# Alexandre-nk-Perdereau/video-fingerprint

Measured on NVIDIA B200. Metric: fingerprint videos/s (64 frames@64^2), higher is better.
Workload: dtype bf16

## Files before the change

### video_fingerprint_b200/csrc/ffn_kernel.cuh

```cuda
#pragma once
#include "epilogues.cuh"
#include "sm100_primitives.cuh"

namespace vfp {

constexpr int kFfnHidden = 1024;
constexpr int kFfnChunk = 256;
constexpr int kFfnChunks = kFfnHidden / kFfnChunk;
constexpr int kFfnActWarps = 16;
constexpr int kFfnThreads = 64 + 32 * kFfnActWarps;

#ifdef VFP_FFN_TRACE
__device__ long long g_ffn_trace[8192];
__device__ unsigned int g_ffn_trace_n = 0;
#define FFN_TRACE_DECL(role) int trace_i = 0; const int trace_role = (role); (void)trace_i; (void)trace_role
#define FFN_TRACE(tag) do { if (blockIdx.x == 0 && trace_i < 1024) { g_ffn_trace[(trace_role * 1024 + trace_i) * 2] = (tag); g_ffn_trace[(trace_role * 1024 + trace_i) * 2 + 1] = clock64(); ++trace_i; } } while (0)
#else
#define FFN_TRACE_DECL(role)
#define FFN_TRACE(tag)
#endif

template <int SLOTS>
struct FfnSmem {
  static constexpr int kA0 = 0;
  static constexpr int kRing = kA0 + 4 * 16384;
  static constexpr int kH = kRing + SLOTS * 16384;
  static constexpr int kBias = kH + 4 * 16384;
  static constexpr int kBars = kBias + 5 * 1024;
  static constexpr int kTotal = kBars + 512 + 1024;
};

struct FfnParams {
  alignas(64) CUtensorMap tmap_x;
  alignas(64) CUtensorMap tmap_w1;
  alignas(64) CUtensorMap tmap_w2;
  alignas(64) CUtensorMap tmap_out;
  const float* b1;
  const float* b2;
  int M;
  int pair_tiles;
};

template <int SLOTS>
__global__ void __launch_bounds__(kFfnThreads, 1) ffn_pair_kernel(const __grid_constant__ FfnParams p) {
  using L = FfnSmem<SLOTS>;
  static_assert(L::kTotal <= 232448, "ffn kernel shared memory");
  extern __shared__ uint8_t smem_raw[];
  uint8_t* smem = smem_raw + ((1024u - (smem_u32(smem_raw) & 1023u)) & 1023u);
  uint8_t* a0 = smem + L::kA0;
  uint8_t* ring = smem + L::kRing;
  uint8_t* hbuf = smem + L::kH;
  float* sbias = reinterpret_cast<float*>(smem + L::kBias);
  uint64_t* bars = reinterpret_cast<uint64_t*>(smem + L::kBars);
  uint64_t* full = bars;
  uint64_t* empty = bars + SLOTS;
  uint64_t* a0_full = bars + 2 * SLOTS;
  uint64_t* a0_empty = a0_full + 1;
  uint64_t* d1_full = a0_full + 2;
  uint64_t* d1_empty = a0_full + 3;
  uint64_t* h_full = a0_full + 4;
  uint64_t* h_empty = a0_full + 5;
  uint64_t* d2_full = a0_full + 6;
  uint64_t* d2_empty = a0_full + 7;
  uint32_t* tmem_slot = reinterpret_cast<uint32_t*>(a0_full + 8);

  const int warp = threadIdx.x >> 5, lane = threadIdx.x & 31;
  const uint32_t crank = cluster_ctarank();
  const bool leader = crank == 0;
  const int pair = blockIdx.x >> 1, n_pairs = gridDim.x >> 1;
  const int my_tiles = p.pair_tiles > pair ? (p.pair_tiles - pair + n_pairs - 1) / n_pairs : 0;
  const int n_chunks = my_tiles * kFfnChunks;
  pdl_launch_dependents();

  if (warp == 0 && lane == 0) {
    tma_prefetch_desc(&p.tmap_x);
    tma_prefetch_desc(&p.tmap_w1);
    tma_prefetch_desc(&p.tmap_w2);
    tma_prefetch_desc(&p.tmap_out);
    for (int i = 0; i < SLOTS; ++i) {
      mbar_init(&full[i], 1);
      mbar_init(&empty[i], 1);
    }
    mbar_init(a0_full, 1);
    mbar_init(a0_empty, 1);
    mbar_init(d1_full, 1);
    mbar_init(d1_empty, 2 * kFfnActWarps);
    mbar_init(h_full, 2 * kFfnActWarps);
    mbar_init(h_empty, 1);
    mbar_init(d2_full, 1);
    mbar_init(d2_empty, 2 * kFfnActWarps);
    fence_mbar_init();
  }
  if (warp == 1) {
    tmem_alloc_2cta(tmem_slot, 512);
    tmem_relinquish_2cta();
  }
  uint32_t* sbias_h = reinterpret_cast<uint32_t*>(sbias);
  for (int i = threadIdx.x; i < kFfnHidden / 2; i += kFfnThreads) {
    const __half2 h = __floats2half2_rn(__ldg(p.b1 + 2 * i), __ldg(p.b1 + 2 * i + 1));
    sbias_h[i] = *reinterpret_cast<const uint32_t*>(&h);
  }
  for (int i = threadIdx.x; i < 256; i += kFfnThreads) sbias[kFfnHidden + i] = __ldg(p.b2 + i);
  tc_fence_before();
  __syncthreads();
  cluster_sync_all();
  tc_fence_after();
  const uint32_t tmem_base = *tmem_slot;
  pdl_wait();

  if (warp == 0) {
    if (lane == 0) {
      int slot = 0;
      uint32_t ph = 0, a_ph = 0;
      const uint32_t a0_full_leader = mapa_u32(a0_full, 0);
      auto load_w = [&](const CUtensorMap* map, int k_col, int row0) {
        mbar_wait(&empty[slot], ph ^ 1);
        if (leader) mbar_arrive_expect_tx(&full[slot], 2 * 16384);
        tma_load_2d_2cta(map, mapa_u32(&full[slot], 0), ring + slot * 16384, k_col, row0 + (int)crank * 128);
        if (++slot == SLOTS) { slot = 0; ph ^= 1; }
      };
      auto load_g1 = [&](int n) {
        const int c = n % kFfnChunks;
        if (c == 0) {
          const int tile = pair + (n / kFfnChunks) * n_pairs;
          mbar_wait(a0_empty, a_ph ^ 1);
          a_ph ^= 1;
          if (leader) mbar_arrive_expect_tx(a0_full, 2 * 4 * 16384);
          for (int kb = 0; kb < 4; ++kb) tma_load_2d_2cta(&p.tmap_x, a0_full_leader, a0 + kb * 16384, kb * 64, (tile * 2 + (int)crank) * 128);
        }
        for (int kb = 0; kb < 4; ++kb) load_w(&p.tmap_w1, kb * 64, c * kFfnChunk);
      };
      auto load_g2 = [&](int n) {
        const int c = n % kFfnChunks;
        for (int kb = 0; kb < 4; ++kb) load_w(&p.tmap_w2, c * kFfnChunk + kb * 64, 0);
      };
      if (n_chunks > 0) load_g1(0);
      for (int n = 0; n < n_chunks; ++n) {
        if (n + 1 < n_chunks) load_g1(n + 1);
// ... 21 lines not shown
        mbar_wait(d1_empty, d1e_ph ^ 1);
        d1e_ph ^= 1;
        tc_fence_after();
        FFN_TRACE(101);
        for (int kb = 0; kb < 4; ++kb) {
          mbar_wait(&full[slot], ph);
          tc_fence_after();
          const uint64_t adesc = umma_smem_desc_kmajor<128>(a0_addr + kb * 16384);
          const uint64_t bdesc = umma_smem_desc_kmajor<128>(smem_u32(ring + slot * 16384));
#pragma unroll
          for (int k = 0; k < 4; ++k) umma_bf16_2cta(tmem_base, adesc + 2 * k, bdesc + 2 * k, idesc, (kb | k) != 0 ? 1u : 0u);
          commit_slot();
        }
        umma_commit_2cta(d1_full, 3);
        FFN_TRACE(102);
        if (c == kFfnChunks - 1) umma_commit_2cta(a0_empty, 3);
      };
      auto gemm2 = [&](int n) {
        const int c = n % kFfnChunks;
        if (c == 0) {
          mbar_wait(d2_empty, d2e_ph ^ 1);
          d2e_ph ^= 1;
        }
        FFN_TRACE(110);
        mbar_wait(h_full, hf_ph);
        hf_ph ^= 1;
        tc_fence_after();
        FFN_TRACE(111);
        for (int kb = 0; kb < 4; ++kb) {
          mbar_wait(&full[slot], ph);
          tc_fence_after();
// ... 52 lines not shown
      tc_fence_before();
      __syncwarp();
      if (lane == 0) mbar_arrive_cluster(d2_empty_leader);
      fence_proxy_async_smem();
      __syncwarp();
      if (lane == 0) {
        const int grow0 = (tile * 2 + (int)crank) * 128 + q * 32;
        tma_store_2d(&p.tmap_out, stage, cq * 64, grow0);
        tma_store_2d(&p.tmap_out, stage + 2048, cq * 64 + 32, grow0);
        tma_store_commit();
        tma_store_wait_read<0>();
      }
      asm volatile("bar.sync 1, %0;" ::"n"(32 * kFfnActWarps) : "memory");
    };

    for (int n = 0; n < n_chunks; ++n) {
      const int c = n % kFfnChunks;
      if (warp == 2 && lane == 0) FFN_TRACE(200);
      mbar_wait(d1_full, d1f_ph);
      d1f_ph ^= 1;
      tc_fence_after();
      if (warp == 2 && lane == 0) FFN_TRACE(201);
      uint32_t packed[32];
      {
        uint32_t va[32], vb[32];
        tmem_ld_32x32(lane_addr + cq * 64, va);
        tmem_ld_32x32(lane_addr + cq * 64 + 32, vb);
        tmem_ld_wait();
        if (warp == 2 && lane == 0) FFN_TRACE(203);
        tc_fence_before();
        __syncwarp();
        if (lane == 0) mbar_arrive_cluster(d1_empty_leader);
#pragma unroll
        for (int cc = 0; cc < 2; ++cc) {
          uint32_t(&v)[32] = cc ? vb : va;
          const uint32_t* bias = sbias_h + (c * kFfnChunk + cq * 64 + cc * 32) / 2;
// ... 41 lines not shown
```

### video_fingerprint_b200/csrc/sm100_primitives.cuh

```cuda
#pragma once
#include <cuda.h>
#include <cuda_runtime.h>
#include <cuda_bf16.h>
#include <stdint.h>

namespace vfp {

__device__ __forceinline__ uint32_t smem_u32(const void* p) {
  return static_cast<uint32_t>(__cvta_generic_to_shared(p));
}

__device__ __forceinline__ bool elect_one() {
  uint32_t pred = 0;
  asm volatile(
      "{\n\t"
      ".reg .pred P;\n\t"
      "elect.sync _|P, 0xffffffff;\n\t"
      "selp.u32 %0, 1, 0, P;\n\t"
      "}\n"
      : "=r"(pred));
  return pred != 0;
}

__device__ __forceinline__ void pdl_launch_dependents() { asm volatile("griddepcontrol.launch_dependents;" ::: "memory"); }
// ... 181 lines not shown
      "l"(adesc), "l"(bdesc), "r"(idesc), "r"(accumulate)
      : "memory");
}
__device__ __forceinline__ void umma_commit_2cta(uint64_t* bar, uint16_t cta_mask) {
  asm volatile("tcgen05.commit.cta_group::2.mbarrier::arrive::one.shared::cluster.multicast::cluster.b64 [%0], %1;" ::"r"(smem_u32(bar)),
               "h"(cta_mask)
               : "memory");
}

__device__ __forceinline__ void tma_prefetch_l2_2d(const CUtensorMap* m, int c0, int c1) {
  asm volatile("cp.async.bulk.prefetch.tensor.2d.L2.global.tile [%0, {%1, %2}];" ::"l"(reinterpret_cast<uint64_t>(m)), "r"(c0),
               "r"(c1)
               : "memory");
}

__device__ __forceinline__ void tma_store_2d(const CUtensorMap* m, const void* src, int c0, int c1) {
  asm volatile("cp.async.bulk.tensor.2d.global.shared::cta.bulk_group [%0, {%2, %3}], [%1];" ::"l"(
                   reinterpret_cast<uint64_t>(m)),
               "r"(smem_u32(src)), "r"(c0), "r"(c1)
               : "memory");
}
__device__ __forceinline__ void tma_store_commit() { asm volatile("cp.async.bulk.commit_group;" ::: "memory"); }
template <int N>
__device__ __forceinline__ void tma_store_wait_read() {
  asm volatile("cp.async.bulk.wait_group.read %0;" ::"n"(N) : "memory");
}

__device__ __forceinline__ void tmem_alloc(uint32_t* slot_in_smem, uint32_t ncols) {
  asm volatile("tcgen05.alloc.cta_group::1.sync.aligned.shared::cta.b32 [%0], %1;" ::"r"(smem_u32(slot_in_smem)),
               "r"(ncols)
// ... 116 lines not shown
```

### video_fingerprint_b200/csrc/stem_common.cuh

```cuda
#pragma once
#include "conv1_kernel.cuh"
#include "epilogues.cuh"

namespace vfp {

constexpr int kStemThreads = 768;
constexpr int kStemEpiWarp0 = 4, kStemEpiWarps = 8;
constexpr int kStemABuf = 9 * 16 * 128;
constexpr int kStemUnitBytes = 2 * kStemABuf;
constexpr int kStemWBlocks = 5;
constexpr int kStemRawSlotBytes = 8192;
constexpr int kStemTilePitch = 72;
constexpr int kStemTileBytes = 29184;
static_assert((67 * kStemTilePitch + 8) * 6 <= kStemTileBytes, "HWC tile");

template <int N> __device__ __forceinline__ void setmaxnreg_inc() { asm volatile("setmaxnreg.inc.sync.aligned.u32 %0;" ::"n"(N)); }
template <int N> __device__ __forceinline__ void setmaxnreg_dec() { asm volatile("setmaxnreg.dec.sync.aligned.u32 %0;" ::"n"(N)); }

__device__ __forceinline__ uint32_t relu_pack_bf16x2(float lo, float hi) {
  uint32_t d;
  asm("cvt.rn.relu.bf16x2.f32 %0, %1, %2;" : "=r"(d) : "f"(hi), "f"(lo));
  return d;
}
__device__ __forceinline__ void bulk_copy_g2s(void* dst, const void* src, uint32_t bytes, uint64_t* bar) {
  asm volatile("cp.async.bulk.shared::cluster.global.mbarrier::complete_tx::bytes [%0], [%1], %2, [%3];" ::"r"(smem_u32(dst)),
               "l"(reinterpret_cast<uint64_t>(src)), "r"(bytes), "r"(smem_u32(bar))
               : "memory");
}
__device__ __forceinline__ void bulk_prefetch_l2(const void* src, uint32_t bytes) {
  asm volatile("cp.async.bulk.prefetch.L2.global [%0], %1;" ::"l"(reinterpret_cast<uint64_t>(src)), "r"(bytes) : "memory");
}
__device__ __forceinline__ uint32_t u8x2_to_bf16x2(uint32_t lo, uint32_t hi) {
  return pack_bf16x2((float)lo * (1.0f / 255.0f), (float)hi * (1.0f / 255.0f));
}

__device__ __forceinline__ void stem_transpose_frame(const uint8_t* const (&pl)[3], uint8_t* tile, int frame_dtype, int ltid,
                                                     int n_threads) {
  if (frame_dtype == kFrameBF16) {
    for (int i = ltid; i < 512; i += n_threads) {
      const int h = i >> 3, w0 = (i & 7) * 8;
      const uint4 a = *reinterpret_cast<const uint4*>(pl[0] + (h * 64 + w0) * 2);
      const uint4 b = *reinterpret_cast<const uint4*>(pl[1] + (h * 64 + w0) * 2);
      const uint4 c = *reinterpret_cast<const uint4*>(pl[2] + (h * 64 + w0) * 2);
      uint4* dst = reinterpret_cast<uint4*>(tile + (h + 2) * (kStemTilePitch * 6) + (w0 + 8) * 6);
      uint4 o0, o1, o2;
// ... 53 lines not shown
```

### video_fingerprint_b200/csrc/token_kernels.cuh

```cuda
#pragma once
#include "sm100_primitives.cuh"
#include "epilogues.cuh"

namespace vfp {

constexpr int kDim = 256;
constexpr int kHeads = 8;
constexpr int kHeadDim = 32;

struct FrameSrc {
  unsigned long long addr;
  long long pitch;
};

__global__ void token_map_kernel(const int* __restrict__ cu, const FrameSrc* __restrict__ src, int n_clips, int n_tokens,
                                 int* __restrict__ tok_pos, int* __restrict__ tok_len, unsigned long long* __restrict__ frame_addr) {
  pdl_launch_dependents();
  pdl_wait();
  const int t = blockIdx.x * blockDim.x + threadIdx.x;
  if (t >= n_tokens) return;
  int lo = 0, hi = n_clips;
  while (hi - lo > 1) {
    const int mid = (lo + hi) >> 1;
    if (cu[mid] <= t) lo = mid; else hi = mid;
// ... 3 lines not shown
  tok_len[t] = cu[lo + 1] - cu[lo];
  const FrameSrc s = src[lo];
  frame_addr[t] = s.addr + (unsigned long long)((long long)pos * s.pitch);
}

__global__ void __launch_bounds__(256)
add_layernorm_bf16_kernel(float* __restrict__ x, const __nv_bfloat16* __restrict__ delta ,
                          const __nv_bfloat16* __restrict__ delta2 ,
                          const float* __restrict__ gamma, const float* __restrict__ beta, __nv_bfloat16* __restrict__ y,
                          int n_tokens, int write_x) {
  pdl_launch_dependents();
  pdl_wait();
  const int warp = (blockIdx.x * blockDim.x + threadIdx.x) >> 5;
  const int lane = threadIdx.x & 31;
  if (warp >= n_tokens) return;
  float4* xr = reinterpret_cast<float4*>(x + (size_t)warp * kDim) + lane * 2;
  const float4 a = xr[0], b = xr[1];
  float v[8] = {a.x, a.y, a.z, a.w, b.x, b.y, b.z, b.w};
  if (delta) {
    const uint4 d = reinterpret_cast<const uint4*>(delta + (size_t)warp * kDim)[lane];
    const __nv_bfloat162* dp = reinterpret_cast<const __nv_bfloat162*>(&d);
#pragma unroll
    for (int e = 0; e < 4; ++e) {
      const float2 f = __bfloat1622float2(dp[e]);
      v[2 * e] += f.x;
      v[2 * e + 1] += f.y;
    }
    if (delta2) {
      const uint4 d2 = reinterpret_cast<const uint4*>(delta2 + (size_t)warp * kDim)[lane];
      const __nv_bfloat162* dp2 = reinterpret_cast<const __nv_bfloat162*>(&d2);
#pragma unroll
      for (int e = 0; e < 4; ++e) {
        const float2 f = __bfloat1622float2(dp2[e]);
        v[2 * e] += f.x;
        v[2 * e + 1] += f.y;
      }
    }
    if (write_x) {
      xr[0] = make_float4(v[0], v[1], v[2], v[3]);
      xr[1] = make_float4(v[4], v[5], v[6], v[7]);
    }
  }
  float s = 0.f;
#pragma unroll
  for (int i = 0; i < 8; ++i) s += v[i];
#pragma unroll
  for (int o = 16; o > 0; o >>= 1) s += __shfl_xor_sync(0xffffffffu, s, o);
  const float mean = s * (1.0f / kDim);
  float q = 0.f;
#pragma unroll
  for (int i = 0; i < 8; ++i) { v[i] -= mean; q += v[i] * v[i]; }
#pragma unroll
  for (int o = 16; o > 0; o >>= 1) q += __shfl_xor_sync(0xffffffffu, q, o);
  const float rstd = rsqrtf(q * (1.0f / kDim) + 1e-5f);
  const float4 g0 = __ldg(reinterpret_cast<const float4*>(gamma) + lane * 2);
  const float4 g1 = __ldg(reinterpret_cast<const float4*>(gamma) + lane * 2 + 1);
  const float4 b0 = __ldg(reinterpret_cast<const float4*>(beta) + lane * 2);
  const float4 b1 = __ldg(reinterpret_cast<const float4*>(beta) + lane * 2 + 1);
  uint4 o;
  o.x = pack_bf16x2(v[0] * rstd * g0.x + b0.x, v[1] * rstd * g0.y + b0.y);
  o.y = pack_bf16x2(v[2] * rstd * g0.z + b0.z, v[3] * rstd * g0.w + b0.w);
  o.z = pack_bf16x2(v[4] * rstd * g1.x + b1.x, v[5] * rstd * g1.y + b1.y);
  o.w = pack_bf16x2(v[6] * rstd * g1.z + b1.z, v[7] * rstd * g1.w + b1.w);
  reinterpret_cast<uint4*>(y + (size_t)warp * kDim)[lane] = o;
}

__global__ void __launch_bounds__(256)
add_convert_bf16_kernel(float* __restrict__ x, const __nv_bfloat16* __restrict__ delta ,
                        const __nv_bfloat16* __restrict__ delta2 , __nv_bfloat16* __restrict__ xbf,
                        long long n8) {
  pdl_launch_dependents();
  pdl_wait();
  const long long i = (long long)blockIdx.x * blockDim.x + threadIdx.x;
  if (i >= n8) return;
  float4* xr = reinterpret_cast<float4*>(x) + 2 * i;
  const float4 a = xr[0], b = xr[1];
  float v[8] = {a.x, a.y, a.z, a.w, b.x, b.y, b.z, b.w};
  if (delta) {
    const uint4 d = reinterpret_cast<const uint4*>(delta)[i];
// ... 456 lines not shown
```

### video_fingerprint_b200/csrc/vfp_b200.cu

```cuda
#include "../../include/vfp_b200.h"

#include <math.h>
#include <string.h>

#include <map>
#include <mutex>
#include <string>
#include <vector>

#include "conv1_kernel.cuh"
#include "attention_tc_kernel.cuh"
#include "conv3_ts_kernel.cuh"
#include "ffn_kernel.cuh"
#include "gemm_launch.cuh"
#include "join_kernels.cuh"
#include "metrics_kernels.cuh"
#include "model3d_kernels.cuh"
#include "preprocess_kernels.cuh"
#include "stem_ts_kernel.cuh"
#include "token_kernels.cuh"
#include "topk_kernels.cuh"

using namespace vfp;

namespace {

thread_local std::string g_last_error;

int fail(const std::string& msg) {
  g_last_error = msg;
// ... 186 lines not shown
int prep_f32(vfp_weights* w, const float* src, size_t n, float** dev) {
  std::vector<float> v(src, src + n);
  return upload(w, v, dev);
}

constexpr int64_t kConvPassFrames = 262144;
constexpr int64_t kStemPassFrames = 16384;
int64_t g_conv_pass_frames = 65536;
int64_t g_stem_pass_frames = kStemPassFrames;
int g_fused_stem = 2;
int g_join_prefetch = 16;
int g_attention_tc = 1;
int g_conv3_ts = 1;
int g_pair_gemm = 1;
int g_ffn_mode = 1;
int g_conv_mcast = 0;
int g_join_kernel = 2;
int g_join_symmetric = 1;
int g_join_panel_tiles = 512;

struct TokenWs {
  size_t cu, frame_src, att_items, frame_addr, tok_pos, tok_len, feat, xa, xb, xn, qkv, att, delta, delta2, h, logits, xbf, pooled, pooled_bf, head_h, total;
};
struct ConvWs {
  size_t c1, c2, c3, total;
};
TokenWs token_ws_layout(int64_t F, int64_t C) {
  TokenWs L{};
  size_t off = 0;
  auto take = [&](size_t bytes) {
// ... 71 lines not shown
  int sms = 0;
  if (cudaDeviceGetAttribute(&sms, cudaDevAttrMultiProcessorCount, dev) != cudaSuccess) return 0;
  return sms;
}

int vfp_set_tuning(int key, long long value) {
  if (key == 0 && value >= 64 && value <= kStemPassFrames) { g_stem_pass_frames = value; return 0; }
  if (key == 1 && (value == 0 || value == 2)) { g_fused_stem = (int)value; return 0; }
  if (key == 5 && value >= 0 && value <= 4096) { g_join_prefetch = (int)value; return 0; }
  if (key == 6 && value >= 0 && value <= 4096) { g_topk_prefetch = (int)value; return 0; }
  if (key == 3 && value >= 64 && value <= kConvPassFrames) { g_conv_pass_frames = value; return 0; }
  if (key == 16 && value >= 0 && value <= 1) { g_conv3_ts = (int)value; return 0; }
  if (key == 17 && value >= 0 && value <= 1) { g_attention_tc = (int)value; return 0; }
  if (key == 15 && value >= 0 && value <= 3) { g_pair_gemm = (int)value; return 0; }
  if (key == 14 && value >= 0 && value <= 1) { g_ffn_mode = (int)value; return 0; }
  if (key == 13 && value >= 0 && value <= 3) { g_conv_mcast = (int)value; return 0; }
  if (key == 10 && value >= 0 && value <= 2) { g_join_kernel = (int)value; return 0; }
  if (key == 11 && value >= 0 && value <= 1) { g_join_symmetric = (int)value; return 0; }
  if (key == 12 && value >= 16 && value <= 65536) { g_join_panel_tiles = (int)value; return 0; }
  if (key == 7 && value >= 0 && value <= 1) { pdl_enabled().store((int)value); return 0; }
  if (key == 8 && value >= 0 && value <= 4096) { persistent_cta_limit().store((int)value); return 0; }
  if (key == 9 && value >= 1 && value <= kMaxPipes) { g_forward_pipes = (int)value; return 0; }
  if (key == 2) {
    const int mode = value != 0;
    const unsigned int zero = 0;
    if (cudaMemcpyToSymbol(g_vfp_hang_mode, &mode, sizeof(mode)) != cudaSuccess) return 2;
    if (cudaMemcpyToSymbol(g_vfp_hang_count, &zero, sizeof(zero)) != cudaSuccess) return 2;
    return 0;
  }
  return 1;
// ... 392 lines not shown

  std::vector<int32_t> cu_rel(C + 1);
  for (int i = 0; i <= C; ++i) cu_rel[i] = (int32_t)(cu_host[c0 + i] - f0);
  size_t n_items = 0;
  for (int i = 0; i < C; ++i) n_items += (size_t)(cu_rel[i + 1] - cu_rel[i] + kAttRows - 1) / kAttRows;
  std::vector<uint8_t> tables(L.att_items - L.cu + n_items * 16);
  memcpy(tables.data(), cu_rel.data(), (size_t)(C + 1) * 4);
  memcpy(tables.data() + (L.frame_src - L.cu), src + c0, (size_t)C * sizeof(FrameSrc));
  int32_t* items_host = reinterpret_cast<int32_t*>(tables.data() + (L.att_items - L.cu));
  for (int i = 0; i < C; ++i)
    for (int q = cu_rel[i]; q < cu_rel[i + 1]; q += kAttRows) {
      items_host[0] = q; items_host[1] = cu_rel[i]; items_host[2] = cu_rel[i + 1]; items_host[3] = 0;
      items_host += 4;
    }
  g_prof.mark(-1, st);
  g_prof.launches += 8 + 7 * (unsigned long long)w->n_attn;
  int4* att_items = reinterpret_cast<int4*>(ws + L.att_items);
  VFP_CUDA(cudaMemcpyAsync(d_cu, tables.data(), tables.size(), cudaMemcpyHostToDevice, st));
  VFP_CUDA(launch_kernel(token_map_kernel, dim3((unsigned)((F + 255) / 256)), dim3(256), 0, st, (const int*)d_cu, d_src, C, (int)F,
                         tok_pos, tok_len, frame_addr));
  g_prof.mark(kStMisc, st);

  for (int64_t s0 = 0; s0 < F; s0 += g_conv_pass_frames) {
    const int64_t n = std::min<int64_t>(g_conv_pass_frames, F - s0);
    if (int rc = encode_frames_pass(w, frame_addr + s0, frame_dtype, fused_ok, n, feat + s0 * 256, conv_ws, st))
      return rc;
  }
  auto token_gemm = [&](const __nv_bfloat16* A, int64_t M, int K, const CUtensorMap& tb, int N, const EpiBiasAct::Params& ep) -> int {
    CUtensorMap tma;
    if (make_tmap_rows_bf16(&tma, A, (uint64_t)M, (uint64_t)K, (uint64_t)K, 128, 64)) return fail("tensor map encode failed (tokens)");
    GemmShape s = plain_shape(M, N, K, 256, 64, 32);
// ... 42 lines not shown
      const int grid = std::min(tp.n_tiles, 2 * persistent_grid());
      VFP_CUDA(launch_kernel(temporal_conv_tma_kernel, dim3((unsigned)grid), dim3(kTc2Threads), kTc2SmemBytes, st, tp));
    }
    g_prof.mark(kStTemporalConv, st);
  }
  const unsigned ln_grid = (unsigned)((F * 32 + 255) / 256);
  VFP_CUDA(ensure_dynamic_smem(reinterpret_cast<const void*>(attention_fa_kernel), kAttSmemBytes));
  AttnTcParams atc{};
  if (g_attention_tc) {
    if (make_tmap_rows_bf16(&atc.tmap_qkv, qkv, (uint64_t)F, 3 * kDim, 3 * kDim, 64, 64)) return fail("tensor map encode failed (attention)");
    atc.items = att_items; atc.out = att; atc.n_units = (int)n_items * 4;
    VFP_CUDA(ensure_dynamic_smem(reinterpret_cast<const void*>(attention_tc_kernel), kAtcSmemBytes));
  }
  for (int b = 0; b < w->n_attn; ++b) {
    const AttnBlockWeights& a = w->attn[b];
    VFP_CUDA(launch_kernel(add_layernorm_bf16_kernel, dim3(ln_grid), dim3(256), 0, st, xa, b > 0 ? delta : nullptr, b > 0 ? delta_f : nullptr, a.ln1_w, a.ln1_b, xn, (int)F, 1));
    g_prof.mark(kStLayerNorm, st);
    if (token_gemm_bf16(xn, F, kDim, a.tm_qkv, 3 * kDim, a.bqkv, 0, qkv, &a.tm_qkv_h)) return 1;
    g_prof.mark(kStQkv, st);
    if (g_attention_tc) {
      const int grid = std::min(atc.n_units, 2 * persistent_grid());
      VFP_CUDA(launch_kernel(attention_tc_kernel, dim3((unsigned)grid), dim3(kAtcThreads), kAtcSmemBytes, st, atc));
    } else {
      VFP_CUDA(launch_kernel(attention_fa_kernel, dim3((unsigned)n_items), dim3(kAttThreads), kAttSmemBytes, st, qkv, att_items, att, (int)F));
    }
    g_prof.mark(kStAttention, st);
    if (token_gemm_bf16(att, F, kDim, a.tm_o, kDim, a.bo, 0, delta, &a.tm_o_h)) return 1;
    g_prof.mark(kStOutProj, st);
    VFP_CUDA(launch_kernel(add_layernorm_bf16_kernel, dim3(ln_grid), dim3(256), 0, st, xa, delta, (const __nv_bfloat16*)nullptr, a.ln2_w, a.ln2_b, xn, (int)F, 0));
    g_prof.mark(kStLayerNorm, st);
    if (g_ffn_mode == 0) {
      if (token_gemm_bf16(xn, F, kDim, a.tm_w1, 4 * kDim, a.b1, 2, hbuf)) return 1;
      g_prof.mark(kStMlp1, st);
      if (token_gemm_bf16(hbuf, F, 4 * kDim, a.tm_w2, kDim, a.b2, 0, delta_f)) return 1;
      g_prof.mark(kStMlp2, st);
    } else {
      FfnParams fp{};
      if (make_tmap_rows_bf16(&fp.tmap_x, xn, (uint64_t)F, kDim, kDim, 128, 64)) return fail("tensor map encode failed (feed-forward)");
      fp.tmap_w1 = a.tm_w1_ffn; fp.tmap_w2 = a.tm_w2_ffn;
      if (make_tmap_out(&fp.tmap_out, delta_f, (uint64_t)F, kDim, true)) return fail("tensor map encode failed (feed-forward out)");
      fp.b1 = a.b1; fp.b2 = a.b2; fp.M = (int)F; fp.pair_tiles = (int)((F + 255) / 256);
      const int grid = 2 * std::min(fp.pair_tiles, persistent_grid() / 2);
      VFP_CUDA(ensure_dynamic_smem(reinterpret_cast<const void*>(ffn_pair_kernel<5>), FfnSmem<5>::kTotal));
      VFP_CUDA(launch_kernel_cluster(2, ffn_pair_kernel<5>, dim3(grid), dim3(kFfnThreads), FfnSmem<5>::kTotal, st, fp));
      g_prof.mark(kStFfn, st);
    }
  }
  VFP_CUDA(launch_kernel(add_convert_bf16_kernel, dim3((unsigned)((F * kDim / 8 + 255) / 256)), dim3(256), 0, st, xa, w->n_attn > 0 ? delta : nullptr,
                         w->n_attn > 0 ? delta_f : nullptr, xbf, (long long)(F * kDim / 8)));
  if (features_out)
    VFP_CUDA(cudaMemcpyAsync(features_out + (size_t)f0 * kDim, xa, (size_t)F * kDim * 4, cudaMemcpyDeviceToDevice, st));
  {
    CUtensorMap tma;
    if (make_tmap_rows_bf16(&tma, xbf, (uint64_t)F, kDim, kDim, 128, 64)) return fail("tensor map encode failed (pool in)");
    EpiBiasActTma<false>::Params ep{};
    if (make_tmap_out(&ep.tmap_out, logits, (uint64_t)F, kDim, false)) return fail("tensor map encode failed (pool logits)");
    ep.bias = w->bpool; ep.N = kDim; ep.act = 1;
    GemmShape s = plain_shape(F, kDim, kDim, 256, 64, 32);
    VFP_CUDA((launch_gemm_bres<256, 64, 2, 4, EpiBiasActTma<false>>(tma, w->tm_pool, s, ep, st)));
// ... 672 lines not shown
```

Baseline: 296,500.

## Fuse LayerNorm into QKV GEMM and feed-forward kernels

Adds a persistent 2-CTA LN+QKV kernel whose normaliser warps compute the residual-add LayerNorm directly into swizzled shared-memory A tiles, replacing the separate LayerNorm launch and QKV GEMM. The feed-forward kernel gains an LN template variant in which the activation warps normalise the next tile into the A buffer instead of loading a precomputed xn via TMA. A shared row-LayerNorm helper is factored out. This removes two LayerNorm launches and the xn round trip per block, but puts normalisation work on the epilogue warps and may serialise LN with the GEMM.

```diff
diff --git a/video_fingerprint_b200/csrc/ffn_kernel.cuh b/video_fingerprint_b200/csrc/ffn_kernel.cuh
--- a/video_fingerprint_b200/csrc/ffn_kernel.cuh
+++ b/video_fingerprint_b200/csrc/ffn_kernel.cuh
@@ -1,5 +1,6 @@
 #pragma once
 #include "epilogues.cuh"
+#include "layernorm_row.cuh"
 #include "sm100_primitives.cuh"
 
 namespace vfp {
@@ -26,7 +27,8 @@
   static constexpr int kRing = kA0 + 4 * 16384;
   static constexpr int kH = kRing + SLOTS * 16384;
   static constexpr int kBias = kH + 4 * 16384;
-  static constexpr int kBars = kBias + 5 * 1024;
+  static constexpr int kLn = kBias + 5 * 1024;
+  static constexpr int kBars = kLn + 2 * 1024;
   static constexpr int kTotal = kBars + 512 + 1024;
 };
 
@@ -37,11 +39,15 @@
   alignas(64) CUtensorMap tmap_out;
   const float* b1;
   const float* b2;
+  const float* x;
+  const __nv_bfloat16* delta;
+  const float* ln_w;
+  const float* ln_b;
   int M;
   int pair_tiles;
 };
 
-template <int SLOTS>
+template <int SLOTS, bool LN>
 __global__ void __launch_bounds__(kFfnThreads, 1) ffn_pair_kernel(const __grid_constant__ FfnParams p) {
   using L = FfnSmem<SLOTS>;
   static_assert(L::kTotal <= 232448, "ffn kernel shared memory");
@@ -51,6 +57,7 @@
   uint8_t* ring = smem + L::kRing;
   uint8_t* hbuf = smem + L::kH;
   float* sbias = reinterpret_cast<float*>(smem + L::kBias);
+  float* sln = reinterpret_cast<float*>(smem + L::kLn);
   uint64_t* bars = reinterpret_cast<uint64_t*>(smem + L::kBars);
   uint64_t* full = bars;
   uint64_t* empty = bars + SLOTS;
@@ -73,7 +80,7 @@
   pdl_launch_dependents();
 
   if (warp == 0 && lane == 0) {
-    tma_prefetch_desc(&p.tmap_x);
+    if constexpr (!LN) tma_prefetch_desc(&p.tmap_x);
     tma_prefetch_desc(&p.tmap_w1);
     tma_prefetch_desc(&p.tmap_w2);
     tma_prefetch_desc(&p.tmap_out);
@@ -81,7 +88,7 @@
       mbar_init(&full[i], 1);
       mbar_init(&empty[i], 1);
     }
-    mbar_init(a0_full, 1);
+    mbar_init(a0_full, LN ? 2 * kFfnActWarps : 1);
     mbar_init(a0_empty, 1);
     mbar_init(d1_full, 1);
     mbar_init(d1_empty, 2 * kFfnActWarps);
@@ -101,6 +108,8 @@
     sbias_h[i] = *reinterpret_cast<const uint32_t*>(&h);
   }
   for (int i = threadIdx.x; i < 256; i += kFfnThreads) sbias[kFfnHidden + i] = __ldg(p.b2 + i);
+  if constexpr (LN)
+    for (int i = threadIdx.x; i < 512; i += kFfnThreads) sln[i] = __ldg(i < 256 ? p.ln_w + i : p.ln_b + i - 256);
   tc_fence_before();
   __syncthreads();
   cluster_sync_all();
@@ -121,7 +130,14 @@
       };
       auto load_g1 = [&](int n) {
         const int c = n % kFfnChunks;
-        if (c == 0) {
+        if (LN && c == 0) {
+          const long long next0 = (long long)((pair + (n / kFfnChunks + 1) * n_pairs) * 2 + (int)crank) * 128;
+          if (next0 < p.M) {
+            const uint32_t rows = (uint32_t)min(128LL, (long long)p.M - next0);
+            bulk_prefetch_l2(p.x + next0 * 256, rows * 1024);
+            bulk_prefetch_l2(p.delta + next0 * 256, rows * 512);
+          }
+        } else if (c == 0) {
           const int tile = pair + (n / kFfnChunks) * n_pairs;
           mbar_wait(a0_empty, a_ph ^ 1);
           a_ph ^= 1;
@@ -173,7 +189,7 @@
         }
         umma_commit_2cta(d1_full, 3);
         FFN_TRACE(102);
-        if (c == kFfnChunks - 1) umma_commit_2cta(a0_empty, 3);
+        if (!LN && c == kFfnChunks - 1) umma_commit_2cta(a0_empty, 3);
       };
       auto gemm2 = [&](int n) {
         const int c = n % kFfnChunks;
@@ -256,12 +272,22 @@
       asm volatile("bar.sync 1, %0;" ::"n"(32 * kFfnActWarps) : "memory");
     };
 
+    auto normalise_tile = [&](int tile) {
+      ln_rows_to_tile<8>(a0, warp - 2, kFfnActWarps, (long long)(tile * 2 + (int)crank) * 128, p.M, const_cast<float*>(p.x), p.delta,
+                            nullptr, 0, sln, sln + 256, lane);
+      fence_proxy_async_smem();
+      __syncwarp();
+      if (lane == 0) mbar_arrive_cluster(mapa_u32(a0_full, 0));
+    };
+    if (LN && n_chunks > 0) normalise_tile(pair);
+
     for (int n = 0; n < n_chunks; ++n) {
       const int c = n % kFfnChunks;
       if (warp == 2 && lane == 0) FFN_TRACE(200);
       mbar_wait(d1_full, d1f_ph);
       d1f_ph ^= 1;
       tc_fence_after();
+      if (LN && c == kFfnChunks - 1 && n + 1 < n_chunks) normalise_tile(pair + (n / kFfnChunks + 1) * n_pairs);
       if (warp == 2 && lane == 0) FFN_TRACE(201);
       uint32_t packed[32];
       {
diff --git a/video_fingerprint_b200/csrc/layernorm_row.cuh b/video_fingerprint_b200/csrc/layernorm_row.cuh
--- /dev/null
+++ b/video_fingerprint_b200/csrc/layernorm_row.cuh
@@ -0,0 +1,95 @@
+#pragma once
+#include "epilogues.cuh"
+#include "sm100_primitives.cuh"
+
+namespace vfp {
+
+constexpr int kLnDim = 256;
+
+struct LnRowIn {
+  float4 a, b;
+  uint4 d, d2;
+};
+
+__device__ __forceinline__ LnRowIn ln_row_load(const float* x, const __nv_bfloat16* delta ,
+                                               const __nv_bfloat16* delta2 , long long row, int lane) {
+  LnRowIn in;
+  const float4* xr = reinterpret_cast<const float4*>(x + row * kLnDim) + lane * 2;
+  in.a = xr[0];
+  in.b = xr[1];
+  in.d = in.d2 = make_uint4(0u, 0u, 0u, 0u);
+  if (delta) {
+    in.d = reinterpret_cast<const uint4*>(delta + row * kLnDim)[lane];
+    if (delta2) in.d2 = reinterpret_cast<const uint4*>(delta2 + row * kLnDim)[lane];
+  }
+  return in;
+}
+
+__device__ __forceinline__ uint4 ln_row_finish(const LnRowIn& in, bool has_delta, bool has_delta2, float* x_row, int write_x,
+                                               const float* gamma, const float* beta, int lane) {
+  float v[8] = {in.a.x, in.a.y, in.a.z, in.a.w, in.b.x, in.b.y, in.b.z, in.b.w};
+  if (has_delta) {
+    const __nv_bfloat162* dp = reinterpret_cast<const __nv_bfloat162*>(&in.d);
+#pragma unroll
+    for (int e = 0; e < 4; ++e) {
+      const float2 f = __bfloat1622float2(dp[e]);
+      v[2 * e] += f.x;
+      v[2 * e + 1] += f.y;
+    }
+    if (has_delta2) {
+      const __nv_bfloat162* dp2 = reinterpret_cast<const __nv_bfloat162*>(&in.d2);
+#pragma unroll
+      for (int e = 0; e < 4; ++e) {
+        const float2 f = __bfloat1622float2(dp2[e]);
+        v[2 * e] += f.x;
+        v[2 * e + 1] += f.y;
+      }
+    }
+    if (write_x) {
+      float4* xr = reinterpret_cast<float4*>(x_row) + lane * 2;
+      xr[0] = make_float4(v[0], v[1], v[2], v[3]);
+      xr[1] = make_float4(v[4], v[5], v[6], v[7]);
+    }
+  }
+  float s = 0.f;
+#pragma unroll
+  for (int i = 0; i < 8; ++i) s += v[i];
+#pragma unroll
+  for (int o = 16; o > 0; o >>= 1) s += __shfl_xor_sync(0xffffffffu, s, o);
+  const float mean = s * (1.0f / kLnDim);
+  float q = 0.f;
+#pragma unroll
+  for (int i = 0; i < 8; ++i) { v[i] -= mean; q += v[i] * v[i]; }
+#pragma unroll
+  for (int o = 16; o > 0; o >>= 1) q += __shfl_xor_sync(0xffffffffu, q, o);
+  const float rstd = rsqrtf(q * (1.0f / kLnDim) + 1e-5f);
+  const float4 g0 = reinterpret_cast<const float4*>(gamma)[lane * 2];
+  const float4 g1 = reinterpret_cast<const float4*>(gamma)[lane * 2 + 1];
+  const float4 b0 = reinterpret_cast<const float4*>(beta)[lane * 2];
+  const float4 b1 = reinterpret_cast<const float4*>(beta)[lane * 2 + 1];
+  uint4 o;
+  o.x = pack_bf16x2(v[0] * rstd * g0.x + b0.x, v[1] * rstd * g0.y + b0.y);
+  o.y = pack_bf16x2(v[2] * rstd * g0.z + b0.z, v[3] * rstd * g0.w + b0.w);
+  o.z = pack_bf16x2(v[4] * rstd * g1.x + b1.x, v[5] * rstd * g1.y + b1.y);
+  o.w = pack_bf16x2(v[6] * rstd * g1.z + b1.z, v[7] * rstd * g1.w + b1.w);
+  return o;
+}
+
+template <int kRows>
+__device__ __forceinline__ void ln_rows_to_tile(uint8_t* tile, int row0, int step, long long grow0, long long M, float* x,
+                                                const __nv_bfloat16* delta, const __nv_bfloat16* delta2, int write_x,
+                                                const float* gamma, const float* beta, int lane) {
+  const bool has_delta = delta != nullptr, has_delta2 = has_delta && delta2 != nullptr;
+  uint8_t* col = tile + (lane >> 3) * 16384;
+  const int piece = lane & 7;
+#pragma unroll 2
+  for (int i = 0; i < kRows; ++i) {
+    const int r = row0 + i * step;
+    const long long g = grow0 + r;
+    uint4 o = make_uint4(0u, 0u, 0u, 0u);
+    if (g < M) o = ln_row_finish(ln_row_load(x, delta, delta2, g, lane), has_delta, has_delta2, x + g * kLnDim, write_x, gamma, beta, lane);
+    *reinterpret_cast<uint4*>(col + r * 128 + ((piece ^ (r & 7)) << 4)) = o;
+  }
+}
+
+}
diff --git a/video_fingerprint_b200/csrc/ln_qkv_kernel.cuh b/video_fingerprint_b200/csrc/ln_qkv_kernel.cuh
--- /dev/null
+++ b/video_fingerprint_b200/csrc/ln_qkv_kernel.cuh
@@ -0,0 +1,217 @@
+#pragma once
+#include "epilogues.cuh"
+#include "layernorm_row.cuh"
+#include "sm100_primitives.cuh"
+
+namespace vfp {
+
+constexpr int kLnQkvChunks = 3;
+constexpr int kLnQkvNormWarps = 8;
+constexpr int kLnQkvOutWarps = 8;
+constexpr int kLnQkvThreads = 64 + 32 * (kLnQkvNormWarps + kLnQkvOutWarps);
+
+template <int SLOTS>
+struct LnQkvSmem {
+  static constexpr int kA = 0;
+  static constexpr int kRing = kA + 2 * 4 * 16384;
+  static constexpr int kStage = kRing + SLOTS * 16384;
+  static constexpr int kBias = kStage + kLnQkvOutWarps * 4096;
+  static constexpr int kBars = kBias + (768 + 512) * 4;
+  static constexpr int kTotal = kBars + 512 + 1024;
+};
+
+struct LnQkvParams {
+  alignas(64) CUtensorMap tmap_w;
+  alignas(64) CUtensorMap tmap_out;
+  float* x;
+  const __nv_bfloat16* delta;
+  const __nv_bfloat16* delta_f;
+  const float* ln_w;
+  const float* ln_b;
+  const float* bias;
+  int M;
+  int pair_tiles;
+};
+
+template <int SLOTS>
+__global__ void __launch_bounds__(kLnQkvThreads, 1) ln_qkv_pair_kernel(const __grid_constant__ LnQkvParams p) {
+  using L = LnQkvSmem<SLOTS>;
+  static_assert(L::kTotal <= 232448, "ln_qkv kernel shared memory");
+  extern __shared__ uint8_t smem_raw[];
+  uint8_t* smem = smem_raw + ((1024u - (smem_u32(smem_raw) & 1023u)) & 1023u);
+  uint8_t* ring = smem + L::kRing;
+  float* sbias = reinterpret_cast<float*>(smem + L::kBias);
+  float* sln = sbias + 768;
+  uint64_t* bars = reinterpret_cast<uint64_t*>(smem + L::kBars);
+  uint64_t* full = bars;
+  uint64_t* empty = bars + SLOTS;
+  uint64_t* a_full = bars + 2 * SLOTS;
+  uint64_t* a_empty = a_full + 2;
+  uint64_t* d_full = a_full + 4;
+  uint64_t* d_empty = a_full + 6;
+  uint32_t* tmem_slot = reinterpret_cast<uint32_t*>(a_full + 8);
+
+  const int warp = threadIdx.x >> 5, lane = threadIdx.x & 31;
+  const uint32_t crank = cluster_ctarank();
+  const bool leader = crank == 0;
+  const int pair = blockIdx.x >> 1, n_pairs = gridDim.x >> 1;
+  const int my_tiles = p.pair_tiles > pair ? (p.pair_tiles - pair + n_pairs - 1) / n_pairs : 0;
+  const int n_chunks = my_tiles * kLnQkvChunks;
+  pdl_launch_dependents();
+
+  if (warp == 0 && lane == 0) {
+    tma_prefetch_desc(&p.tmap_w);
+    tma_prefetch_desc(&p.tmap_out);
+    for (int i = 0; i < SLOTS; ++i) {
+      mbar_init(&full[i], 1);
+      mbar_init(&empty[i], 1);
+    }
+    for (int i = 0; i < 2; ++i) {
+      mbar_init(&a_full[i], 2 * kLnQkvNormWarps);
+      mbar_init(&a_empty[i], 1);
+      mbar_init(&d_full[i], 1);
+      mbar_init(&d_empty[i], 2 * kLnQkvOutWarps);
+    }
+    fence_mbar_init();
+  }
+  if (warp == 1) {
+    tmem_alloc_2cta(tmem_slot, 512);
+    tmem_relinquish_2cta();
+  }
+  for (int i = threadIdx.x; i < 768; i += kLnQkvThreads) sbias[i] = __ldg(p.bias + i);
+  for (int i = threadIdx.x; i < 512; i += kLnQkvThreads) sln[i] = __ldg(i < 256 ? p.ln_w + i : p.ln_b + i - 256);
+  tc_fence_before();
+  __syncthreads();
+  cluster_sync_all();
+  tc_fence_after();
+  const uint32_t tmem_base = *tmem_slot;
+  pdl_wait();
+
+  if (warp == 0) {
+    if (lane == 0) {
+      int slot = 0;
+      uint32_t ph = 0;
+      for (int n = 0; n < n_chunks; ++n) {
+        const int c = n % kLnQkvChunks;
+        for (int kb = 0; kb < 4; ++kb) {
+          mbar_wait(&empty[slot], ph ^ 1);
+          if (leader) mbar_arrive_expect_tx(&full[slot], 2 * 16384);
+          tma_load_2d_2cta(&p.tmap_w, mapa_u32(&full[slot], 0), ring + slot * 16384, kb * 64, c * 256 + (int)crank * 128);
+          if (++slot == SLOTS) { slot = 0; ph ^= 1; }
+        }
+      }
+    }
+  } else if (warp == 1) {
+    if (lane == 0 && leader) {
+      constexpr uint32_t idesc = umma_idesc_bf16(256, 256);
+      int slot = 0;
+      uint32_t ph = 0;
+      for (int n = 0; n < n_chunks; ++n) {
+        const int c = n % kLnQkvChunks, t = n / kLnQkvChunks, ab = t & 1, buf = n & 1;
+        if (c == 0) mbar_wait(&a_full[ab], (t >> 1) & 1);
+        mbar_wait(&d_empty[buf], ((n >> 1) & 1) ^ 1);
+        tc_fence_after();
+        const uint32_t a_addr = smem_u32(smem + L::kA + ab * 65536);
+        for (int kb = 0; kb < 4; ++kb) {
+          mbar_wait(&full[slot], ph);
+          tc_fence_after();
+          const uint64_t adesc = umma_smem_desc_kmajor<128>(a_addr + kb * 16384);
+          const uint64_t bdesc = umma_smem_desc_kmajor<128>(smem_u32(ring + slot * 16384));
+#pragma unroll
+          for (int k = 0; k < 4; ++k) umma_bf16_2cta(tmem_base + buf * 256, adesc + 2 * k, bdesc + 2 * k, idesc, (kb | k) != 0 ? 1u : 0u);
+          umma_commit_2cta(&empty[slot], 3);
+          if (++slot == SLOTS) { slot = 0; ph ^= 1; }
+        }
+        umma_commit_2cta(&d_full[buf], 3);
+        if (c == kLnQkvChunks - 1) umma_commit_2cta(&a_empty[ab], 3);
+      }
+    }
+  } else if (warp < 2 + kLnQkvNormWarps) {
+    const int nw = warp - 2;
+    const uint32_t a_full_leader0 = mapa_u32(&a_full[0], 0);
+    for (int t = 0; t < my_tiles; ++t) {
+      const int ab = t & 1;
+      const long long grow0 = (long long)((pair + t * n_pairs) * 2 + (int)crank) * 128;
+      if (nw == 0 && lane == 0) {
+        const long long next0 = grow0 + (long long)n_pairs * 256;
+        if (next0 < p.M) {
+          const uint32_t rows = (uint32_t)min(128LL, (long long)p.M - next0);
+          bulk_prefetch_l2(p.x + next0 * 256, rows * 1024);
+          if (p.delta) bulk_prefetch_l2(p.delta + next0 * 256, rows * 512);
+          if (p.delta && p.delta_f) bulk_prefetch_l2(p.delta_f + next0 * 256, rows * 512);
+        }
+      }
+      mbar_wait(&a_empty[ab], ((t >> 1) & 1) ^ 1);
+      ln_rows_to_tile<128 / kLnQkvNormWarps>(smem + L::kA + ab * 65536, nw, kLnQkvNormWarps, grow0, p.M, p.x, p.delta, p.delta_f, 1,
+                                             sln, sln + 256, lane);
+      fence_proxy_async_smem();
+      __syncwarp();
+      if (lane == 0) mbar_arrive_cluster(a_full_leader0 + ab * 8);
+    }
+  } else {
+    const int ow = warp - 2 - kLnQkvNormWarps;
+    const int q = warp & 3;
+    const int ch = ow >> 2;
+    const uint32_t lane_addr = tmem_base + (static_cast<uint32_t>(q * 32) << 16);
+    const uint32_t d_empty_leader0 = mapa_u32(&d_empty[0], 0);
+    uint8_t* stage = smem + L::kStage + ow * 4096;
+    for (int n = 0; n < n_chunks; ++n) {
+      const int c = n % kLnQkvChunks, buf = n & 1;
+      const int tile = pair + (n / kLnQkvChunks) * n_pairs;
+      mbar_wait(&d_full[buf], (n >> 1) & 1);
+      tc_fence_after();
+#pragma unroll 1
+      for (int h = 0; h < 2; ++h) {
+        if (lane == 0) tma_store_wait_read<0>();
+        __syncwarp();
+#pragma unroll
+        for (int s = 0; s < 2; ++s) {
+          const int col = ch * 128 + h * 64 + s * 32;
+          uint32_t v[32];
+          tmem_ld_32x32(lane_addr + buf * 256 + col, v);
+          tmem_ld_wait();
+          if (h == 1 && s == 1) {
+            tc_fence_before();
+            __syncwarp();
+            if (lane == 0) mbar_arrive_cluster(d_empty_leader0 + buf * 8);
+          }
+          const float* bias = sbias + c * 256 + col;
+          uint8_t* r0 = stage + s * 2048 + lane * 64;
+          const int s64 = (lane >> 1) & 3;
+#pragma unroll
+          for (int piece = 0; piece < 4; ++piece) {
+            const float4 ba = *reinterpret_cast<const float4*>(bias + 8 * piece);
+            const float4 bc = *reinterpret_cast<const float4*>(bias + 8 * piece + 4);
+            uint4 o;
+            o.x = pack_bf16x2(__uint_as_float(v[8 * piece + 0]) + ba.x, __uint_as_float(v[8 * piece + 1]) + ba.y);
+            o.y = pack_bf16x2(__uint_as_float(v[8 * piece + 2]) + ba.z, __uint_as_float(v[8 * piece + 3]) + ba.w);
+            o.z = pack_bf16x2(__uint_as_float(v[8 * piece + 4]) + bc.x, __uint_as_float(v[8 * piece + 5]) + bc.y);
+            o.w = pack_bf16x2(__uint_as_float(v[8 * piece + 6]) + bc.z, __uint_as_float(v[8 * piece + 7]) + bc.w);
+            *reinterpret_cast<uint4*>(r0 + ((piece ^ s64) << 4)) = o;
+          }
+        }
+        fence_proxy_async_smem();
+        __syncwarp();
+        if (lane == 0) {
+          const int grow0 = (tile * 2 + (int)crank) * 128 + q * 32;
+          const int col0 = c * 256 + ch * 128 + h * 64;
+          tma_store_2d(&p.tmap_out, stage, col0, grow0);
+          tma_store_2d(&p.tmap_out, stage + 2048, col0 + 32, grow0);
+          tma_store_commit();
+        }
+      }
+    }
+    if (lane == 0) tma_store_wait_read<0>();
+  }
+
+  __syncwarp();
+  tc_fence_before();
+  __syncthreads();
+  cluster_sync_all();
+  if (warp == 1) {
+    tc_fence_after();
+    tmem_dealloc_2cta(tmem_base, 512);
+  }
+}
+
+}
diff --git a/video_fingerprint_b200/csrc/sm100_primitives.cuh b/video_fingerprint_b200/csrc/sm100_primitives.cuh
--- a/video_fingerprint_b200/csrc/sm100_primitives.cuh
+++ b/video_fingerprint_b200/csrc/sm100_primitives.cuh
@@ -219,6 +219,10 @@
                : "memory");
 }
 
+__device__ __forceinline__ void bulk_prefetch_l2(const void* p, uint32_t bytes) {
+  asm volatile("cp.async.bulk.prefetch.L2.global [%0], %1;" ::"l"(reinterpret_cast<uint64_t>(p)), "r"(bytes) : "memory");
+}
+
 __device__ __forceinline__ void tma_store_2d(const CUtensorMap* m, const void* src, int c0, int c1) {
   asm volatile("cp.async.bulk.tensor.2d.global.shared::cta.bulk_group [%0, {%2, %3}], [%1];" ::"l"(
                    reinterpret_cast<uint64_t>(m)),
diff --git a/video_fingerprint_b200/csrc/stem_common.cuh b/video_fingerprint_b200/csrc/stem_common.cuh
--- a/video_fingerprint_b200/csrc/stem_common.cuh
+++ b/video_fingerprint_b200/csrc/stem_common.cuh
@@ -26,9 +26,6 @@
   asm volatile("cp.async.bulk.shared::cluster.global.mbarrier::complete_tx::bytes [%0], [%1], %2, [%3];" ::"r"(smem_u32(dst)),
                "l"(reinterpret_cast<uint64_t>(src)), "r"(bytes), "r"(smem_u32(bar))
                : "memory");
-}
-__device__ __forceinline__ void bulk_prefetch_l2(const void* src, uint32_t bytes) {
-  asm volatile("cp.async.bulk.prefetch.L2.global [%0], %1;" ::"l"(reinterpret_cast<uint64_t>(src)), "r"(bytes) : "memory");
 }
 __device__ __forceinline__ uint32_t u8x2_to_bf16x2(uint32_t lo, uint32_t hi) {
   return pack_bf16x2((float)lo * (1.0f / 255.0f), (float)hi * (1.0f / 255.0f));
diff --git a/video_fingerprint_b200/csrc/token_kernels.cuh b/video_fingerprint_b200/csrc/token_kernels.cuh
--- a/video_fingerprint_b200/csrc/token_kernels.cuh
+++ b/video_fingerprint_b200/csrc/token_kernels.cuh
@@ -1,10 +1,12 @@
 #pragma once
 #include "sm100_primitives.cuh"
 #include "epilogues.cuh"
+#include "layernorm_row.cuh"
 
 namespace vfp {
 
 constexpr int kDim = 256;
+static_assert(kDim == kLnDim, "LayerNorm rows are one token");
 constexpr int kHeads = 8;
 constexpr int kHeadDim = 32;
 
@@ -41,55 +43,9 @@
   const int warp = (blockIdx.x * blockDim.x + threadIdx.x) >> 5;
   const int lane = threadIdx.x & 31;
   if (warp >= n_tokens) return;
-  float4* xr = reinterpret_cast<float4*>(x + (size_t)warp * kDim) + lane * 2;
-  const float4 a = xr[0], b = xr[1];
-  float v[8] = {a.x, a.y, a.z, a.w, b.x, b.y, b.z, b.w};
-  if (delta) {
-    const uint4 d = reinterpret_cast<const uint4*>(delta + (size_t)warp * kDim)[lane];
-    const __nv_bfloat162* dp = reinterpret_cast<const __nv_bfloat162*>(&d);
-#pragma unroll
-    for (int e = 0; e < 4; ++e) {
-      const float2 f = __bfloat1622float2(dp[e]);
-      v[2 * e] += f.x;
-      v[2 * e + 1] += f.y;
-    }
-    if (delta2) {
-      const uint4 d2 = reinterpret_cast<const uint4*>(delta2 + (size_t)warp * kDim)[lane];
-      const __nv_bfloat162* dp2 = reinterpret_cast<const __nv_bfloat162*>(&d2);
-#pragma unroll
-      for (int e = 0; e < 4; ++e) {
-        const float2 f = __bfloat1622float2(dp2[e]);
-        v[2 * e] += f.x;
-        v[2 * e + 1] += f.y;
-      }
-    }
-    if (write_x) {
-      xr[0] = make_float4(v[0], v[1], v[2], v[3]);
-      xr[1] = make_float4(v[4], v[5], v[6], v[7]);
-    }
-  }
-  float s = 0.f;
-#pragma unroll
-  for (int i = 0; i < 8; ++i) s += v[i];
-#pragma unroll
-  for (int o = 16; o > 0; o >>= 1) s += __shfl_xor_sync(0xffffffffu, s, o);
-  const float mean = s * (1.0f / kDim);
-  float q = 0.f;
-#pragma unroll
-  for (int i = 0; i < 8; ++i) { v[i] -= mean; q += v[i] * v[i]; }
-#pragma unroll
-  for (int o = 16; o > 0; o >>= 1) q += __shfl_xor_sync(0xffffffffu, q, o);
-  const float rstd = rsqrtf(q * (1.0f / kDim) + 1e-5f);
-  const float4 g0 = __ldg(reinterpret_cast<const float4*>(gamma) + lane * 2);
-  const float4 g1 = __ldg(reinterpret_cast<const float4*>(gamma) + lane * 2 + 1);
-  const float4 b0 = __ldg(reinterpret_cast<const float4*>(beta) + lane * 2);
-  const float4 b1 = __ldg(reinterpret_cast<const float4*>(beta) + lane * 2 + 1);
-  uint4 o;
-  o.x = pack_bf16x2(v[0] * rstd * g0.x + b0.x, v[1] * rstd * g0.y + b0.y);
-  o.y = pack_bf16x2(v[2] * rstd * g0.z + b0.z, v[3] * rstd * g0.w + b0.w);
-  o.z = pack_bf16x2(v[4] * rstd * g1.x + b1.x, v[5] * rstd * g1.y + b1.y);
-  o.w = pack_bf16x2(v[6] * rstd * g1.z + b1.z, v[7] * rstd * g1.w + b1.w);
-  reinterpret_cast<uint4*>(y + (size_t)warp * kDim)[lane] = o;
+  const LnRowIn in = ln_row_load(x, delta, delta2, warp, lane);
+  reinterpret_cast<uint4*>(y + (size_t)warp * kDim)[lane] =
+      ln_row_finish(in, delta != nullptr, delta != nullptr && delta2 != nullptr, x + (size_t)warp * kDim, write_x, gamma, beta, lane);
 }
 
 __global__ void __launch_bounds__(256)
diff --git a/video_fingerprint_b200/csrc/vfp_b200.cu b/video_fingerprint_b200/csrc/vfp_b200.cu
--- a/video_fingerprint_b200/csrc/vfp_b200.cu
+++ b/video_fingerprint_b200/csrc/vfp_b200.cu
@@ -14,6 +14,7 @@
 #include "ffn_kernel.cuh"
 #include "gemm_launch.cuh"
 #include "join_kernels.cuh"
+#include "ln_qkv_kernel.cuh"
 #include "metrics_kernels.cuh"
 #include "model3d_kernels.cuh"
 #include "preprocess_kernels.cuh"
@@ -230,6 +231,7 @@
 int g_conv3_ts = 1;
 int g_pair_gemm = 1;
 int g_ffn_mode = 1;
+int g_token_ln = 1;
 int g_conv_mcast = 0;
 int g_join_kernel = 2;
 int g_join_symmetric = 1;
@@ -331,6 +333,7 @@
   if (key == 17 && value >= 0 && value <= 1) { g_attention_tc = (int)value; return 0; }
   if (key == 15 && value >= 0 && value <= 3) { g_pair_gemm = (int)value; return 0; }
   if (key == 14 && value >= 0 && value <= 1) { g_ffn_mode = (int)value; return 0; }
+  if (key == 18 && value >= 0 && value <= 1) { g_token_ln = (int)value; return 0; }
   if (key == 13 && value >= 0 && value <= 3) { g_conv_mcast = (int)value; return 0; }
   if (key == 10 && value >= 0 && value <= 2) { g_join_kernel = (int)value; return 0; }
   if (key == 11 && value >= 0 && value <= 1) { g_join_symmetric = (int)value; return 0; }
@@ -753,7 +756,8 @@
       items_host += 4;
     }
   g_prof.mark(-1, st);
-  g_prof.launches += 8 + 7 * (unsigned long long)w->n_attn;
+  const bool ln2_separate = !g_token_ln || g_ffn_mode == 0;
+  g_prof.launches += 8 + (unsigned long long)w->n_attn * ((g_token_ln ? 1 : 2) + 2 + (ln2_separate ? 1 : 0) + (g_ffn_mode ? 1 : 2));
   int4* att_items = reinterpret_cast<int4*>(ws + L.att_items);
   VFP_CUDA(cudaMemcpyAsync(d_cu, tables.data(), tables.size(), cudaMemcpyHostToDevice, st));
   VFP_CUDA(launch_kernel(token_map_kernel, dim3((unsigned)((F + 255) / 256)), dim3(256), 0, st, (const int*)d_cu, d_src, C, (int)F,
@@ -826,9 +830,20 @@
   }
   for (int b = 0; b < w->n_attn; ++b) {
     const AttnBlockWeights& a = w->attn[b];
-    VFP_CUDA(launch_kernel(add_layernorm_bf16_kernel, dim3(ln_grid), dim3(256), 0, st, xa, b > 0 ? delta : nullptr, b > 0 ? delta_f : nullptr, a.ln1_w, a.ln1_b, xn, (int)F, 1));
-    g_prof.mark(kStLayerNorm, st);
-    if (token_gemm_bf16(xn, F, kDim, a.tm_qkv, 3 * kDim, a.bqkv, 0, qkv, &a.tm_qkv_h)) return 1;
+    if (g_token_ln) {
+      LnQkvParams lp{};
+      lp.tmap_w = a.tm_qkv_h;
+      if (make_tmap_out(&lp.tmap_out, qkv, (uint64_t)F, 3 * kDim, true)) return fail("tensor map encode failed (qkv out)");
+      lp.x = xa; lp.delta = b > 0 ? delta : nullptr; lp.delta_f = b > 0 ? delta_f : nullptr;
+      lp.ln_w = a.ln1_w; lp.ln_b = a.ln1_b; lp.bias = a.bqkv; lp.M = (int)F; lp.pair_tiles = (int)((F + 255) / 256);
+      const int grid = 2 * std::min(lp.pair_tiles, persistent_grid() / 2);
+      VFP_CUDA(ensure_dynamic_smem(reinterpret_cast<const void*>(ln_qkv_pair_kernel<3>), LnQkvSmem<3>::kTotal));
+      VFP_CUDA(launch_kernel_cluster(2, ln_qkv_pair_kernel<3>, dim3(grid), dim3(kLnQkvThreads), LnQkvSmem<3>::kTotal, st, lp));
+    } else {
+      VFP_CUDA(launch_kernel(add_layernorm_bf16_kernel, dim3(ln_grid), dim3(256), 0, st, xa, b > 0 ? delta : nullptr, b > 0 ? delta_f : nullptr, a.ln1_w, a.ln1_b, xn, (int)F, 1));
+      g_prof.mark(kStLayerNorm, st);
+      if (token_gemm_bf16(xn, F, kDim, a.tm_qkv, 3 * kDim, a.bqkv, 0, qkv, &a.tm_qkv_h)) return 1;
+    }
     g_prof.mark(kStQkv, st);
     if (g_attention_tc) {
       const int grid = std::min(atc.n_units, 2 * persistent_grid());
@@ -839,8 +854,10 @@
     g_prof.mark(kStAttention, st);
     if (token_gemm_bf16(att, F, kDim, a.tm_o, kDim, a.bo, 0, delta, &a.tm_o_h)) return 1;
     g_prof.mark(kStOutProj, st);
-    VFP_CUDA(launch_kernel(add_layernorm_bf16_kernel, dim3(ln_grid), dim3(256), 0, st, xa, delta, (const __nv_bfloat16*)nullptr, a.ln2_w, a.ln2_b, xn, (int)F, 0));
-    g_prof.mark(kStLayerNorm, st);
+    if (ln2_separate) {
+      VFP_CUDA(launch_kernel(add_layernorm_bf16_kernel, dim3(ln_grid), dim3(256), 0, st, xa, delta, (const __nv_bfloat16*)nullptr, a.ln2_w, a.ln2_b, xn, (int)F, 0));
+      g_prof.mark(kStLayerNorm, st);
+    }
     if (g_ffn_mode == 0) {
       if (token_gemm_bf16(xn, F, kDim, a.tm_w1, 4 * kDim, a.b1, 2, hbuf)) return 1;
       g_prof.mark(kStMlp1, st);
@@ -848,13 +865,19 @@
       g_prof.mark(kStMlp2, st);
     } else {
       FfnParams fp{};
-      if (make_tmap_rows_bf16(&fp.tmap_x, xn, (uint64_t)F, kDim, kDim, 128, 64)) return fail("tensor map encode failed (feed-forward)");
       fp.tmap_w1 = a.tm_w1_ffn; fp.tmap_w2 = a.tm_w2_ffn;
       if (make_tmap_out(&fp.tmap_out, delta_f, (uint64_t)F, kDim, true)) return fail("tensor map encode failed (feed-forward out)");
       fp.b1 = a.b1; fp.b2 = a.b2; fp.M = (int)F; fp.pair_tiles = (int)((F + 255) / 256);
       const int grid = 2 * std::min(fp.pair_tiles, persistent_grid() / 2);
-      VFP_CUDA(ensure_dynamic_smem(reinterpret_cast<const void*>(ffn_pair_kernel<5>), FfnSmem<5>::kTotal));
-      VFP_CUDA(launch_kernel_cluster(2, ffn_pair_kernel<5>, dim3(grid), dim3(kFfnThreads), FfnSmem<5>::kTotal, st, fp));
+      if (ln2_separate) {
+        if (make_tmap_rows_bf16(&fp.tmap_x, xn, (uint64_t)F, kDim, kDim, 128, 64)) return fail("tensor map encode failed (feed-forward)");
+        VFP_CUDA(ensure_dynamic_smem(reinterpret_cast<const void*>(ffn_pair_kernel<5, false>), FfnSmem<5>::kTotal));
+        VFP_CUDA(launch_kernel_cluster(2, ffn_pair_kernel<5, false>, dim3(grid), dim3(kFfnThreads), FfnSmem<5>::kTotal, st, fp));
+      } else {
+        fp.x = xa; fp.delta = delta; fp.ln_w = a.ln2_w; fp.ln_b = a.ln2_b;
+        VFP_CUDA(ensure_dynamic_smem(reinterpret_cast<const void*>(ffn_pair_kernel<5, true>), FfnSmem<5>::kTotal));
+        VFP_CUDA(launch_kernel_cluster(2, ffn_pair_kernel<5, true>, dim3(grid), dim3(kFfnThreads), FfnSmem<5>::kTotal, st, fp));
+      }
       g_prof.mark(kStFfn, st);
     }
   }
```

Result: slower. 292,300, median of 6 (-1.4%).
